# ktzsh/object-tracking

Measured on AMD Instinct MI355X. Metric: frames/sec detect+track @416x416, higher is better.
Workload: dtype f32; 1 GPU; BASELINE.json configs[2]: MultiObjDetTracker (YOLOv2 C=12 + ConvLSTM2D(512) + 1x1 + decode/NMS + track ids), 48 clips x 30 frames per GPU per step, 416x416 uint8; the synthetic head is calibrated to 32 CANDIDATE boxes per frame, of which about 20 survive NMS (config.boxes_per_frame: measured).  The step computes the model's TRACKING output, the one MultiObjDetTracker.predict reads (MultiObjDetTrac; parallelism=clip-shard x1

## Files before the change

### object_tracking_amd/csrc/conv3_h2.hip

```cpp
#include "dt_internal.h"
#include <type_traits>

typedef _Float16 c3_h8 __attribute__((ext_vector_type(8)));
typedef _Float16 c3_h4 __attribute__((ext_vector_type(4)));
typedef float c3_f16 __attribute__((ext_vector_type(16)));
typedef float c3_f4 __attribute__((ext_vector_type(4)));
typedef unsigned c3_u4 __attribute__((ext_vector_type(4)));
typedef unsigned c3_u2 __attribute__((ext_vector_type(2)));
typedef __attribute__((address_space(3))) void c3_lptr_t;
typedef const __attribute__((address_space(1))) void c3_gptr_t;

constexpr int C3_PW = 18;
#define C3_THREADS 256
#define C3_NS 3

template <int N>
__device__ __forceinline__ void c3_wait_vm() { __builtin_amdgcn_s_waitcnt(0x0f70 | (N & 15) | ((N >> 4) << 14)); }

__device__ __forceinline__ void c3_mfma(c3_f16 &c, const c3_u4 &w, const c3_u4 &a)
{
    c = __builtin_amdgcn_mfma_f32_32x32x16_f16(__builtin_bit_cast(c3_h8, a), __builtin_bit_cast(c3_h8, w), c, 0, 0, 0);
}

template <int WN, bool POOL, bool FUSE = false>
// ... 337 lines not shown
                            const float mx = fmaxf(fmaxf(acc[j][i][r], acc[j][i][r + 1]), fmaxf(acc[j][i][r + 8], acc[j][i][r + 9]));
                            const int x2 = (cur.tx0 >> 1) + 4 * (q >> 1) + 2 * gl + (q & 1);
                            if (nok && y2 < H2 && x2 < W2) {
                                if (p.amax_out) out_am = fmaxf(out_am, fabsf(mx));
                                __builtin_nontemporal_store(mx, p.out2 + (((long long)cur.b * H2 + y2) * W2 + x2) * p.out2_ld + cur.n0 + nl);
                            }
                        }
                    }
                }
            }
        }
        if (!has_next) break;
        __builtin_amdgcn_s_waitcnt(0xc07f);
        __builtin_amdgcn_s_barrier();
        patch_store();
        if (last_chunk && nxt.n0 != cur.n0)
            for (int i = tid; i < BN; i += C3_THREADS) btab[i] = (nxt.n0 + i < p.N) ? p.bias[nxt.n0 + i] : 0.0f;
        item = nitem;
        cur = nxt;
    }
    if (p.amax_out) dt_amax_publish(p.amax_out, out_am);
}

bool conv3_h2_usable(const Conv3H2Args &a)
{
    return a.Cin % 32 == 0 && a.Cin >= 32 && a.N >= 64 && a.N % 64 == 0 && a.Np % 64 == 0 && a.in_ld % 4 == 0 && (reinterpret_cast<uintptr_t>(a.in) & 15) == 0 &&
           a.w && a.pscale && a.amax && a.bias && a.zeros && (a.out != nullptr) != (a.out2 != nullptr) && (!a.out2 || !((a.H | a.W) & 1)) &&
           (!a.w1 || (a.N == 128 && a.out && a.pscale1 && a.bias1 && a.N1 > 0 && a.N1 <= 64 && a.Np1 >= 64 && a.Np1 % 32 == 0));
}
double conv3_h2_flops(const Conv3H2Args &a)
{
    const bool wide = a.N % 128 == 0;
    const int th = wide ? 8 : 16;
    const double tiles = (double)a.B * ((a.H + th - 1) / th) * ((a.W + 15) / 16);
    return 6.0 * tiles * th * 16 * (9.0 * a.Cin * a.N + (a.w1 ? (double)a.N * 64 : 0.0));
}

template <int WN, bool POOL, bool FUSE = false>
static int c3_launch(hipStream_t st, const Conv3H2Args &a, int cus)
{
    constexpr int TH = 16 / WN, BN = 64 * WN;
    const size_t lds = (size_t)4 * (TH + 2) * C3_PW * 32 + (size_t)C3_NS * 4 * BN * 32 + BN * 4 + (FUSE ? 68 * 4 : 0);
    static PerDeviceOnce attr;
    if (attr.ensure(nullptr, [&](int) {
            return hipFuncSetAttribute(reinterpret_cast<const void *>(conv3_h2_kernel<WN, POOL, FUSE>), hipFuncAttributeMaxDynamicSharedMemorySize, (int)lds) != hipSuccess;
        }))
        return 1;
    Conv3H2Args p = a;
    p.tiles_y = (a.H + TH - 1) / TH;
    p.tiles_x = (a.W + 15) / 16;
    const long long items = (long long)a.B * p.tiles_x * p.tiles_y * ((a.N + BN - 1) / BN);
    long long grid = 2ll * cus;
    if (grid > items) grid = items;
    hipLaunchKernelGGL((conv3_h2_kernel<WN, POOL, FUSE>), dim3((unsigned)grid), dim3(C3_THREADS), lds, st, p);
    return hipGetLastError() == hipSuccess ? 0 : 1;
}

int launch_conv3_h2(hipStream_t st, const Conv3H2Args &a)
{
    if (!conv3_h2_usable(a) || a.B <= 0 || a.H <= 0 || a.W <= 0) return 2;
    static int cu_of[64];
    static PerDeviceOnce once;
    int dev = 0;
    if (once.ensure(&dev, [&](int d) {
            int n = 0;
            if (hipDeviceGetAttribute(&n, hipDeviceAttributeMultiprocessorCount, d) != hipSuccess || n <= 0) return 1;
            cu_of[d] = n;
            return 0;
        }))
        return 1;
    const int cus = cu_of[dev];
    const bool wide = a.N % 128 == 0, pool = a.out2 != nullptr;
    if (a.w1) return c3_launch<2, false, true>(st, a, cus);
    if (wide) return pool ? c3_launch<2, true>(st, a, cus) : c3_launch<2, false>(st, a, cus);
    return pool ? c3_launch<1, true>(st, a, cus) : c3_launch<1, false>(st, a, cus);
}
```

### object_tracking_amd/csrc/dt_internal.h

```cpp
#pragma once
#include <hip/hip_runtime.h>

#include <atomic>
#include <cstdint>
#include <cstdio>
#include <map>
#include <mutex>
#include <functional>
#include <string>
#include <type_traits>
#include <vector>

#include "../../include/mi355_dt.h"

struct PerDeviceOnce {
    std::atomic<unsigned long long> mask{0};
    std::mutex mu;
    template <class F> int ensure(int *dev_out, F &&setup)
    {
        int dev = -1;
        if (hipGetDevice(&dev) != hipSuccess || dev < 0 || dev > 63) return 1;
        if (dev_out) *dev_out = dev;
        if ((mask.load(std::memory_order_acquire) >> dev) & 1ull) return 0;
        std::lock_guard<std::mutex> lk(mu);
// ... 101 lines not shown
struct Conv3H2Args {
    const float *in;
    long long in_bs;
    int in_ld;
    int B, H, W, Cin, N, Np;
    const unsigned short *w;
    const float *pscale;
    const unsigned *amax;
    const float *bias;
    float slope;
    float *out;
    long long out_bs;
    int out_ld;
    float *out2;
    int out2_ld;
    const float *zeros;
    unsigned *amax_out;
    int tiles_x, tiles_y;
    const unsigned short *w1;
    const float *pscale1;
    const float *bias1;
    int N1, Np1;
    float slope1;
};
int launch_conv3_h2(hipStream_t st, const Conv3H2Args &a);
bool conv3_h2_usable(const Conv3H2Args &a);
double conv3_h2_flops(const Conv3H2Args &a);
struct GemmS3Args {
    const unsigned short *a;
    const float *a_f32;
    int a_ld;
    const unsigned short *b;
    float *c;
    long long c_ps;
    int P, Mt, Mp, N, Np, K, ldc;
    const unsigned short *ones, *bias_s3;
    int act;
    float slope;
    int half;
    int nt;
    const float *pscale;
    const unsigned *amax;
    const float *bias;
    unsigned *amax_out;
};
#define DT_AMAX_SUB 16
// ... 342 lines not shown
    T *get() const { return p; }
    explicit operator bool() const { return p != nullptr; }
};
static_assert(!std::is_copy_constructible<DevMem<float>>::value && !std::is_copy_assignable<DevMem<float>>::value, "a device allocation has one owner");

struct WinoWeights {
    int ts = 0;
    int cin = 0, npad = 0;
    DevMem<float> u;
    DevMem<unsigned short> s3;
    DevMem<unsigned short> h2;
    DevMem<float> h2_pscale;
};

struct ConvLayer {
    int idx = 0, ks = 0, cin = 0, cout = 0, npad = 0;
    DevMem<float> wt;
    DevMem<unsigned short> wt_s3;
    DevMem<unsigned short> bias_s3;
    DevMem<unsigned short> wt_h2;
    DevMem<float> pscale_h2;
    DevMem<unsigned short> w3_h2;
    DevMem<float> pscale_w3;
    WinoWeights wino;
    WinoWeights wino_alt;
    DevMem<float> fused4s;
    DevMem<float> bias;
    DevMem<float> scale;
    bool scale_has_zero = false;
};

struct Policy {
    int wino = 1;
    int wino_tile = 0;
    int wino_mint = 0;
    double wino_ws_gb = 96.0;
    int mosaic = -1;
    int fused4 = 1;
    int trk_merge = 1;
    int pin = 0;
    int c3h2 = 1;
    int conv_cfg = -1;
    int s3_conv1 = 1;
    int s3 = 1;
    int s3_minrows = 2048;
    int s3_minrows_h2 = 64;
    int s3_h2 = 1;
    int c3fuse = 1;
    int h2_minframes = 12;
    int s3_half = 0;
    int s3_rec_minrows = 512;
    int s3_rec_minrows_h2 = 16;
    int s3_1x1_mink = 256;
    int s3_1x1_minrows = 16384;
    int s3_1x1 = 1;
    int amax_measure = 0;
};

struct StreamTable {
    int n_slots = 0, cap = 0;
    int tcap = 0;
    int row = 0;
    DevMem<float> h, c;
    DevMem<float> boxes;
// ... 1 lines not shown
    DevMem<int> ages;
    DevMem<float> vel;
    DevMem<int> vstamp;
    DevMem<int> hits;
    DevMem<int> hstamp;
    DevMem<int> meta;
    DevMem<int> list;
    std::vector<char> warm;
};

struct TinyStreamTable {
    int n_slots = 0;
    int U = 0;
    DevMem<float> h;
    DevMem<float> c;
    DevMem<int> meta;
    DevMem<int> list;
};

struct dt_ctx {
    std::string err;
    Policy pol;
    int pin_override = -1;
    hipStream_t stream = nullptr;
    int image_h = 0, image_w = 0, cb = 0;
    float dec_anchors_host[64];
    int dec_anchors_n = 0;
    bool det_loaded = false;
    ConvLayer layers[24];
    DevMem<float> s3_ones;
    DevMem<unsigned> amax;
    struct AmaxTag { const float *lo, *hi; int cols, slot; };
    bool h2_small = false;
    std::vector<AmaxTag> amax_tag;
    DevMem<float> conv1_w, conv1_b, lut255;
    DevMem<unsigned> conv1_w3, conv1_w3u8;
    std::vector<float> conv1_hwio32, conv1_scale, conv1_shift;
    bool trk_loaded = false;
    int trk_units = 0, trk_cx = 0 ;
    DevMem<float> trk_wx, trk_bx;
    DevMem<float> trk_wh;
    WinoWeights trk_wx_wino, trk_wh_wino;
    WinoWeights trk_wxm_wino;
    DevMem<float> trk_bx16;
    std::vector<float> conv23_hwio, conv23_bias;
    std::vector<float> trk_hkernel, trk_hbias;
// ... 41 lines not shown
```

### object_tracking_amd/csrc/network.hip

```cpp
#include <algorithm>
#include <cmath>
#include <cstdarg>
#include <cstdlib>
#include <cstring>
#include <thread>

#include "dt_internal.h"

static const float BN_EPS = 1e-3f;
static const float LEAKY = 0.1f;
static char g_static_err[512] = "";

static const int TRUNK[20][5] = {
    {1, 3, 3, 32, 1},      {2, 3, 32, 64, 1},     {3, 3, 64, 128, 0},    {4, 1, 128, 64, 0},
    {5, 3, 64, 128, 1},    {6, 3, 128, 256, 0},   {7, 1, 256, 128, 0},   {8, 3, 128, 256, 1},
    {9, 3, 256, 512, 0},   {10, 1, 512, 256, 0},  {11, 3, 256, 512, 0},  {12, 1, 512, 256, 0},
    {13, 3, 256, 512, 1},  {14, 3, 512, 1024, 0}, {15, 1, 1024, 512, 0}, {16, 3, 512, 1024, 0},
    {17, 1, 1024, 512, 0}, {18, 3, 512, 1024, 0}, {19, 3, 1024, 1024, 0}, {20, 3, 1024, 1024, 0}};

static inline int round_up(int v, int m) { return (v + m - 1) / m * m; }

int dt_fail(dt_ctx *ctx, int code, const char *fmt, ...)
{
    char buf[512];
// ... 204 lines not shown
    if (slot > AMAX_IN && slot < AMAX_TRK) snprintf(tag, sizeof(tag), "conv_%d", slot - AMAX_IN);
    else snprintf(tag, sizeof(tag), "%s", slot == AMAX_TRK ? "trk" : "test");
    ProfScope ps(ctx, "absmax", 0.0, 4.0 * (double)rows * cols, tag);
    if (launch_absmax(ctx->stream, x, rows, cols, ld, 1, 0, s)) { dt_fail(ctx, DT_ERR_DEVICE, "absmax launch failed"); return nullptr; }
    for (const auto &t : ctx->amax_tag)
        if (t.slot == slot) { amax_forget(ctx, t.lo, t.hi - t.lo); break; }
    amax_note(ctx, x, rows * ld, cols, slot);
    return s;
}
static bool h2_wanted(const dt_ctx *ctx) { return ctx->pol.s3 != 0 && ctx->pol.s3_h2 != 0 && !ctx->pol.pin && !ctx->h2_small; }

template <class T> static int upload(dt_ctx *ctx, DevMem<T> &dst, const std::vector<T> &h)
{
    DevMem<T> d;
    HIP_TRY(ctx, d.alloc(h.size()));
    HIP_TRY(ctx, hipMemcpy(d.get(), h.data(), h.size() * sizeof(T), hipMemcpyHostToDevice));
    dst = std::move(d);
    return DT_OK;
}

static const struct { const char *name; int Policy::*field; } k_knobs[] = {
    {"DT_WINO", &Policy::wino}, {"DT_WINO_TILE", &Policy::wino_tile}, {"DT_WINO_MINT", &Policy::wino_mint},
    {"DT_WINO_MOSAIC", &Policy::mosaic}, {"DT_WINO_FUSED4", &Policy::fused4}, {"DT_TRK_MERGE", &Policy::trk_merge},
    {"DT_PIN", &Policy::pin}, {"DT_C3H2", &Policy::c3h2}, {"DT_C3FUSE", &Policy::c3fuse}, {"DT_CONV_CFG", &Policy::conv_cfg},
    {"DT_S3", &Policy::s3}, {"DT_S3_CONV1", &Policy::s3_conv1}, {"DT_S3_MINROWS", &Policy::s3_minrows}, {"DT_S3_H2", &Policy::s3_h2},
    {"DT_H2_MINFRAMES", &Policy::h2_minframes}, {"DT_S3_HALF", &Policy::s3_half}, {"DT_S3_REC_MINROWS", &Policy::s3_rec_minrows},
    {"DT_S3_1X1", &Policy::s3_1x1}, {"DT_S3_1X1_MINK", &Policy::s3_1x1_mink}, {"DT_S3_1X1_MINROWS", &Policy::s3_1x1_minrows},
    {"DT_AMAX_MEASURE", &Policy::amax_measure},
};

static void policy_from_env(Policy &p)
{
    const Policy d;
    for (const auto &k : k_knobs) {
        const char *e = getenv(k.name);
        p.*k.field = e ? atoi(e) : d.*k.field;
    }
    { const char *e = getenv("DT_WINO_WS_GB"); p.wino_ws_gb = e ? atof(e) : d.wino_ws_gb; }
    p.s3_minrows_h2 = getenv("DT_S3_MINROWS") ? p.s3_minrows : d.s3_minrows_h2;
    p.s3_rec_minrows_h2 = getenv("DT_S3_REC_MINROWS") ? p.s3_rec_minrows : d.s3_rec_minrows_h2;
}

static bool policy_equal(const Policy &a, const Policy &b)
{
    for (const auto &k : k_knobs)
        if (a.*k.field != b.*k.field) return false;
    return a.wino_ws_gb == b.wino_ws_gb && a.s3_minrows_h2 == b.s3_minrows_h2 && a.s3_rec_minrows_h2 == b.s3_rec_minrows_h2;
}

static void policy_refresh(dt_ctx *ctx)
{
    Policy p;
    policy_from_env(p);
    if (ctx->pin_override >= 0) p.pin = ctx->pin_override;
    if (p.pin) {
        p.wino = 2; p.mosaic = 1; p.fused4 = 2; p.s3_half = -1;
        if (p.s3) p.s3 = 2;
        p.trk_merge = 0;
    }
    if (!policy_equal(p, ctx->pol)) graphs_clear(ctx);
    ctx->pol = p;
}

extern "C" int dt_abi_version(void) { return 108; }

extern "C" int dt_amax_read(dt_ctx *ctx, int slot, float *h_out)
{
    if (!ctx || !h_out) return dt_fail(ctx, DT_ERR_ARG, "null argument");
    if (slot < 0 || slot >= DT_AMAX_SLOTS) return dt_fail(ctx, DT_ERR_ARG, "max-|x| slot %d out of range [0, %d)", slot, DT_AMAX_SLOTS);
    if (!ctx->amax) return dt_fail(ctx, DT_ERR_STATE, "max-|x| slots not allocated");
    if (ctx->capturing) return dt_fail(ctx, DT_ERR_STATE, "dt_amax_read during graph capture");
    HIP_TRY(ctx, hipStreamSynchronize(ctx->stream));
    unsigned w[DT_AMAX_WORDS];
    HIP_TRY(ctx, hipMemcpy(w, amax_slot(ctx, slot), sizeof(w), hipMemcpyDeviceToHost));
    unsigned v = 0;
    for (int q = 0; q < DT_AMAX_SUB; ++q) v = w[q * DT_AMAX_LINE] > v ? w[q * DT_AMAX_LINE] : v;
    memcpy(h_out, &v, sizeof(v));
// ... 252 lines not shown
            wino_s3_split_host(bias_src[n], t);
            for (int t3 = 0; t3 < 3; ++t3) bs[((size_t)t3 * L.npad + n) * 16] = t[t3];
        }
        if ((rc = upload(ctx, L.bias_s3, bs))) return rc;
        if (!ctx->s3_ones) {
            std::vector<float> ones((size_t)256 * 16, 0.0f);
            for (int r = 0; r < 256; ++r) ones[(size_t)r * 16] = 1.0f;
            if ((rc = upload(ctx, ctx->s3_ones, ones))) return rc;
        }
    }
    if (L.wt_s3 && ctx->pol.s3_h2 != 0) {
        HIP_TRY(ctx, L.wt_h2.alloc(packed.size() * 2));
        HIP_TRY(ctx, L.pscale_h2.alloc(1));
        if (launch_wino_h2_pack(ctx->stream, L.wt.get(), 1, L.npad, cin, 0, amax_slot(ctx, AMAX_PACK), L.wt_h2.get(), L.pscale_h2.get()))
            return dt_fail(ctx, DT_ERR_DEVICE, "fp16-form weight pack launch failed");
        HIP_TRY(ctx, hipStreamSynchronize(ctx->stream));
    }
    if (ks == 3 && (cin == 32 || cin == 64) && cout % 64 == 0 && cout <= 128 && ctx->pol.s3 != 0 && ctx->pol.s3_h2 != 0 && ctx->pol.c3h2 != 0) {
        HIP_TRY(ctx, L.w3_h2.alloc(packed.size() * 2));
        HIP_TRY(ctx, L.pscale_w3.alloc(1));
        if (launch_wino_h2_pack(ctx->stream, L.wt.get(), 1, L.npad, 9 * cin, 0, amax_slot(ctx, AMAX_PACK), L.w3_h2.get(), L.pscale_w3.get()))
            return dt_fail(ctx, DT_ERR_DEVICE, "fp16-form weight pack launch failed");
        HIP_TRY(ctx, hipStreamSynchronize(ctx->stream));
    }
    if (scale) {
        std::vector<float> sc(scale, scale + cout);
        for (float v : sc) L.scale_has_zero |= (v == 0.0f);
        if ((rc = upload(ctx, L.scale, sc))) return rc;
    }
    const bool f4_shape = ((cin == 64 || cin == 128) && cout % 128 == 0 && cout <= 256) || (cin == 32 && cout == 64);
    if (ks == 3 && f4_shape && ctx->pol.wino != 0 && ctx->pol.fused4 != 0) {
        std::vector<float> u36((size_t)36 * L.npad * cin), uf((size_t)36 * cin * cout);
        wino_pack_weights(4, hwio, cin, cout, nullptr, cin, nullptr, L.npad, scale, u36.data());
        wino4s_fused_pack(u36.data(), L.npad, cin, cout, uf.data());
        if ((rc = upload(ctx, L.fused4s, uf))) return rc;
    }
    if (wino_wanted(ctx, ks, cin, cout)) {
        const int ts = wino_tile(ctx, false);
        rc = upload_wino(ctx, L.wino, ts, hwio, cin, cout, nullptr, cin, nullptr, L.npad, scale, ts == 6);
        if (rc) return rc;
        if (ts == 6 && ctx->pol.wino_tile == 0 && cin >= 256) {
            rc = upload_wino(ctx, L.wino_alt, 4, hwio, cin, cout, nullptr, cin, nullptr, L.npad, scale, false);
            if (rc) return rc;
        }
    }
    if ((rc = upload(ctx, L.bias, bias))) return rc;
// ... 333 lines not shown
{
    if (cout <= 64) return CFG_128x64;
    if (ks == 3 && cout % 256 == 0) {
        const long long t256 = (long long)((M + 255) / 256) * (cout / 256);
        const long long t128 = (long long)((M + 127) / 128) * (cout / 128);
        const double e256 = (double)t256 / (double)(((t256 + 255) / 256) * 256);
        const double e128 = (double)t128 / (double)(((t128 + 511) / 512) * 512);
        if (e256 * 1.05 > e128) return CFG_256x256;
    }
    if (ks == 1 && cout >= 128 && (long long)((M + 255) / 256) * ((cout + 127) / 128) >= 4096) return CFG_256x128;
    return CFG_128x128;
}

static bool s3_1x1_eligible(const dt_ctx *ctx, const ConvLayer &L, long long M)
{
    return L.ks == 1 && L.wt_s3 && ctx->pol.s3 != 0 && ctx->pol.s3_1x1 != 0 && L.cin % 32 == 0 && L.cout >= 64 && M < (1ll << 31) - 256 &&
           (ctx->pol.s3 == 2 || (L.cin >= S3_MINK && L.cin >= ctx->pol.s3_1x1_mink && M >= ctx->pol.s3_minrows && M >= ctx->pol.s3_1x1_minrows));
}

enum { CF_S3_1X1, CF_DIRECT_H2, CF_FUSED4, CF_WINO, CF_SPLITK, CF_IGEMM };
struct ConvChoice {
    int form;
    bool h2;
    int cfg, ksplit;
    const WinoWeights *wts; WinoChoice wino;
    bool publishes;
};
static ConvChoice choose_conv(const dt_ctx *ctx, const ConvLayer &L, const float *in, int in_ld, int B, int H, int W, const float *out, int order, int epi, bool has_out2)
{
    ConvChoice c{};
    const bool plain = epi == EPI_PLAIN && order == ORD_LINEAR, pool_even = epi == EPI_POOL && !((H | W) & 1);
    const long long blocks = (long long)B * ((H + 15) / 16) * ((W + 15) / 16) * ((L.cout + 127) / 128);
    if (L.bias_s3 && ctx->s3_ones && plain && !has_out2 && in_ld % 4 == 0 && (reinterpret_cast<uintptr_t>(in) & 15) == 0 &&
        (reinterpret_cast<uintptr_t>(out) & 3) == 0 && s3_1x1_eligible(ctx, L, (long long)B * H * W)) {
        c.form = CF_S3_1X1;
        c.h2 = L.wt_h2 && L.pscale_h2 && L.npad <= 2048 && h2_wanted(ctx);
    }
    else if (L.w3_h2 && L.pscale_w3 && ctx->pol.c3h2 != 0 && h2_wanted(ctx) && in_ld % 4 == 0 && (reinterpret_cast<uintptr_t>(in) & 15) == 0 && (plain || pool_even) &&
             (ctx->pol.c3h2 == 2 || blocks >= C3H2_MIN_BLOCKS))
        c.form = CF_DIRECT_H2;
    else if (L.fused4s && ctx->pol.fused4 != 0 && in_ld % 4 == 0 && (plain || pool_even) &&
             (ctx->pol.fused4 == 2 || (((ctx->pol.fused4 == 1 && L.cin <= 64) || ctx->pol.fused4 == 3) && blocks >= 1024)))
        c.form = CF_FUSED4;
    else if (wino_runs(ctx, L.wino, B, H, W, L.cout) && (plain || epi == EPI_POOL || epi == EPI_POOL_BOTH)) {
        const bool pooled = epi == EPI_POOL || has_out2;
        c.form = CF_WINO; c.wts = &L.wino;
        c.wino = choose_wino(ctx, L.wino, L.cout, B, H, W, pooled, false);
        if (L.wino_alt.u && !ctx->pol.pin) {
            const WinoChoice alt = choose_wino(ctx, L.wino_alt, L.cout, B, H, W, pooled, false);
            const long long t6 = 64ll * ((c.wino.q.Mt + 127) / 128) * ((L.cout + 127) / 128);
            if (c.wino.nt != 2 && t6 <= 4096 && small_gemm_cost(alt.q.Mt, L.cout, 36, nullptr) < small_gemm_cost(c.wino.q.Mt, L.cout, 64, nullptr)) {
                c.wts = &L.wino_alt; c.wino = alt;
            }
        }
    } else {
        const int M = B * H * W;
        c.form = CF_IGEMM; c.ksplit = 1;
        c.cfg = pick_cfg(M, L.cout, L.ks);
        if (plain && c.cfg != CFG_128x64) {
            const int tiles = ((M + 127) / 128) * ((L.cout + 127) / 128), nk = L.ks * L.ks * L.cin / 32;
            if (tiles < 2 * 512 && !ctx->pol.pin) {
                int smax = nk / 6;
                if (smax > 32) smax = 32;
// ... 17 lines not shown
    const ConvLayer &L; const float *in; int in_ld, B, H, W; float *out; int out_ld, order, epi; float slope; float *out2; int out2_ld;
    const char *tag; unsigned *amax_out; int M; double flops, bytes;
};

static int conv_s3_1x1(dt_ctx *ctx, const ConvCall &c, bool h2)
{
    const ConvLayer &L = c.L;
    const long long M = (long long)c.B * c.H * c.W;
    GemmS3Args g{};
    g.a_f32 = c.in; g.a_ld = c.in_ld; g.b = L.wt_s3.get(); g.c = c.out; g.c_ps = 0; g.P = 1; g.Mt = (int)M; g.Mp = (int)((M + 255) / 256 * 256); g.N = L.cout; g.Np = L.npad;
    g.half = ctx->pol.s3_half; g.K = L.cin; g.ldc = c.out_ld; g.ones = reinterpret_cast<const unsigned short *>(ctx->s3_ones.get()); g.bias_s3 = L.bias_s3.get(); g.act = 1; g.slope = c.slope;
    if (h2) {
        g.nt = 2; g.b = L.wt_h2.get(); g.pscale = L.pscale_h2.get(); g.bias = L.bias.get(); g.ones = nullptr; g.bias_s3 = nullptr;
        g.amax = ensure_amax(ctx, c.in, M, L.cin, c.in_ld, amax_in_slot(L));
        if (!g.amax) return DT_ERR_DEVICE;
    }
    g.amax_out = c.amax_out;
    prof_count(ctx, h2 ? "s3_form:f16x2" : "s3_form:bf16x3");
    ProfScope ps(ctx, "conv_gemm_s3", wino_gemm_s3_flops(g), 4.0 * M * L.cin + (h2 ? 4.0 : 6.0) * (double)L.cin * L.cout + 4.0 * (double)M * L.cout, c.tag);
    prof_direct_form(ctx, 2.0 * M * (double)L.cin * L.cout, 4.0 * ((double)M * L.cin + (double)L.cin * L.cout + (double)M * L.cout), DF_S3);
    const int rc = launch_wino_gemm_s3(ctx->stream, g, 0);
    return rc ? dt_fail(ctx, launch_code(rc), "%s: split-bf16 1x1 GEMM launch failed (rc=%d)", c.tag, rc) : DT_OK;
}
static int conv_direct_h2(dt_ctx *ctx, const ConvCall &c, const ConvLayer *L4 = nullptr)
{
    const ConvLayer &L = c.L;
    Conv3H2Args a{};
    a.in = c.in; a.in_bs = (long long)c.H * c.W * c.in_ld; a.in_ld = c.in_ld; a.B = c.B; a.H = c.H; a.W = c.W; a.Cin = L.cin; a.N = L.cout; a.Np = L.npad;
    a.w = L.w3_h2.get(); a.pscale = L.pscale_w3.get(); a.bias = L.bias.get(); a.slope = c.slope;
    if (L4) { a.w1 = L4->wt_h2.get(); a.pscale1 = L4->pscale_h2.get(); a.bias1 = L4->bias.get(); a.N1 = L4->cout; a.Np1 = L4->npad; a.slope1 = c.slope; }
    if (c.epi == EPI_POOL) { a.out2 = c.out; a.out2_ld = c.out_ld; }
    else { a.out = c.out; a.out_ld = c.out_ld; a.out_bs = (long long)c.H * c.W * c.out_ld; }
    a.zeros = ws_get(ctx, "zeros256", 256, true);
    if (!a.zeros) return DT_ERR_DEVICE;
    a.amax = ensure_amax(ctx, c.in, (long long)c.B * c.H * c.W, L.cin, c.in_ld, amax_in_slot(L));
    if (!a.amax) return DT_ERR_DEVICE;
    a.amax_out = c.amax_out;
    if (L4) prof_count(ctx, "conv_direct_h2:fused_1x1");
    const double M = c.M;
    ProfScope ps(ctx, "conv_direct_h2", conv3_h2_flops(a),
                 L4 ? 4.0 * (M * L.cin * 1.41 + M * L4->cout)
                    : 4.0 * ((double)c.B * c.H * c.W * L.cin * (L.cout % 128 ? 1.27 : 1.41) * ((L.cout + 127) / 128) + M * L.cout / (c.epi == EPI_POOL ? 4.0 : 1.0)), c.tag);
    if (L4)
        prof_direct_form(ctx, 2.0 * M * (9.0 * L.cin * L.cout + (double)L4->cin * L4->cout),
                         4.0 * (M * L.cin + 9.0 * L.cin * L.cout + 2.0 * M * L.cout + (double)L4->cin * L4->cout + M * L4->cout), DF_C3H2);
    else prof_direct_form(ctx, c.flops, c.bytes, DF_C3H2);
    const int rc = launch_conv3_h2(ctx->stream, a);
    return rc ? dt_fail(ctx, launch_code(rc), L4 ? "%s: fused direct 3x3 + 1x1 launch failed" : "%s: direct fp16-form 3x3 launch failed", c.tag) : DT_OK;
}
static int conv_fused4(dt_ctx *ctx, const ConvCall &c)
{
    const ConvLayer &L = c.L;
    Wino4FusedArgs f{};
    f.in = c.in; f.in_bs = (long long)c.H * c.W * c.in_ld; f.in_ld = c.in_ld; f.B = c.B; f.H = c.H; f.W = c.W; f.Cin = L.cin; f.N = L.cout;
    f.u = L.fused4s.get(); f.bias = L.bias.get(); f.slope = c.slope;
    if (c.epi == EPI_POOL) { f.out2 = c.out; f.out2_ld = c.out_ld; }
    else { f.out = c.out; f.out_ld = c.out_ld; f.out_bs = (long long)c.H * c.W * c.out_ld; }
    const double tiles = (double)c.B * ((c.H + 3) / 4) * ((c.W + 3) / 4);
    ProfScope ps(ctx, "conv_fused", 2.0 * 36.0 * tiles * L.cin * L.cout,
                 4.0 * ((double)c.B * c.H * c.W * L.cin * 1.27 * ((L.cout + 127) / 128) + (double)c.M * L.cout / (c.epi == EPI_POOL ? 4.0 : 1.0)), c.tag);
    prof_direct_form(ctx, c.flops, c.bytes, DF_FUSED);
// ... 37 lines not shown
            return dt_fail(ctx, DT_ERR_DEVICE, "conv_%d split-K reduce launch failed", L.idx);
        return DT_OK;
    }
    ProfScope ps(ctx, "conv_igemm", c.flops, c.bytes, c.tag);
    a.amax_out = c.amax_out;
    const int rc = launch_igemm(ctx, a, L.ks, c.order, c.epi, cfg);
    return rc ? dt_fail(ctx, launch_code(rc), "conv_%d launch failed (rc=%d)", L.idx, rc) : DT_OK;
}

static int run_conv(dt_ctx *ctx, const ConvLayer &L, const float *in, int in_ld, int B, int H, int W, float *out, int out_ld, int order, int epi, float slope,
                    float *out2 = nullptr, int out2_ld = 0)
{
    const Leaves lv = conv_leaves(epi, out, out_ld, out2, out2_ld, (long long)B * H * W, L.cout);
    amax_forget(ctx, lv);
    const ConvChoice ch = choose_conv(ctx, L, in, in_ld, B, H, W, out, order, epi, out2 != nullptr);
    const int M = B * H * W, K = L.ks * L.ks * L.cin;
    char tag[32];
    snprintf(tag, sizeof(tag), L.idx == 102 ? "tconv_2" : "conv_%d", L.idx);
    const ConvCall c{L, in, in_ld, B, H, W, out, out_ld, order, epi, slope, out2, out2_ld, tag, ch.publishes ? amax_slot(ctx, amax_out_slot(L)) : nullptr, M,
                     2.0 * M * (double)K * L.cout, 4.0 * ((double)M * L.cin + (double)K * L.cout + (double)M * L.cout / (epi == EPI_POOL ? 4.0 : 1.0))};
    int rc = DT_ERR_STATE;
    switch (ch.form) {
    case CF_S3_1X1: rc = conv_s3_1x1(ctx, c, ch.h2); break;
    case CF_DIRECT_H2: rc = conv_direct_h2(ctx, c); break;
    case CF_FUSED4: rc = conv_fused4(ctx, c); break;
    case CF_WINO: rc = conv_wino(ctx, c, *ch.wts, ch.wino); break;
    case CF_SPLITK: case CF_IGEMM: rc = conv_igemm(ctx, c, ch.cfg, ch.ksplit); break;
    }
    if (rc == DT_OK && c.amax_out) amax_note(ctx, lv, amax_out_slot(L));
    return rc;
}

enum { EX_CONV = 0, EX_NORM = 1, EX_ACT = 2, EX_POOL = 3, EX_S2D = 4, EX_CAT = 5 };
struct Extract {
    int idx, kind;
    float *out;
    bool done = false;
};

static int extract_layer(dt_ctx *ctx, const ConvLayer &L, const float *in, int in_ld, int B, int h, int w, Extract &ex)
{
    if (ex.kind == EX_CONV && L.scale && L.scale_has_zero)
        return dt_fail(ctx, DT_ERR_ARG, "conv_%d: a BatchNorm gamma of 0 was folded into the kernel; the raw Conv2D output cannot be recovered", L.idx);
    int rc = run_conv(ctx, L, in, in_ld, B, h, w, ex.out, L.cout, ORD_LINEAR, EPI_PLAIN, ex.kind == EX_ACT ? LEAKY : 1.0f);
    if (rc) return rc;
    if (ex.kind == EX_CONV && L.scale && launch_unfold_bn(ctx->stream, ex.out, (long long)B * h * w, L.cout, L.scale.get(), L.bias.get()))
        return dt_fail(ctx, DT_ERR_DEVICE, "BatchNorm un-fold launch failed");
    ex.done = true;
    return DT_OK;
}

static bool conv34_fusable(const dt_ctx *ctx, const ConvLayer &L3, const ConvLayer &L4, const float *in, int in_ld, int B, int H, int W, const float *out)
{
    return ctx->pol.c3fuse != 0 && L3.ks == 3 && L3.cout == 128 && L4.ks == 1 && L4.cin == 128 && L4.cout <= 64 && L4.wt_h2 && L4.pscale_h2 &&
           choose_conv(ctx, L3, in, in_ld, B, H, W, out, ORD_LINEAR, EPI_PLAIN, false).form == CF_DIRECT_H2;
}
static int run_conv34_fused(dt_ctx *ctx, const ConvLayer &L3, const ConvLayer &L4, const float *in, int in_ld, int B, int H, int W, float *out, int out_ld, float slope)
{
    const Leaves lv = conv_leaves(EPI_PLAIN, out, out_ld, nullptr, 0, (long long)B * H * W, L4.cout);
    amax_forget(ctx, lv);
    char tag[32];
    snprintf(tag, sizeof(tag), "conv_%d", L3.idx);
    const ConvCall c{L3, in, in_ld, B, H, W, out, out_ld, ORD_LINEAR, EPI_PLAIN, slope, nullptr, 0, tag, amax_out_slot(L4) ? amax_slot(ctx, amax_out_slot(L4)) : nullptr, B * H * W, 0.0, 0.0};
    const int rc = conv_direct_h2(ctx, c, &L4);
    if (rc == DT_OK && c.amax_out) amax_note(ctx, lv, amax_out_slot(L4));
    return rc;
}

static int run_trunk(dt_ctx *ctx, int B, float *bufA, float *bufB, float *skip, float *cat, Extract *ex)
{
    const int H = ctx->image_h, W = ctx->image_w;
    float *cur = bufA, *nxt = bufB;
    int h = H / 2, w = W / 2;
    int rc;
    bool cat20 = false;
    for (int li = 1; li < 20; ++li) {
        const int idx = TRUNK[li][0], pool = TRUNK[li][4];
        const ConvLayer &L = ctx->layers[idx];
        if (ex && ex->idx == idx && ex->kind <= EX_ACT) return extract_layer(ctx, L, cur, L.cin, B, h, w, *ex);
        if (idx == 3 && TRUNK[li + 1][0] == 4) {
            const bool ex4 = ex && ex->idx == 4;
            float *out34 = ex4 ? ex->out : nxt;
            if (!(ex4 && ex->kind < EX_ACT) && conv34_fusable(ctx, L, ctx->layers[4], cur, L.cin, B, h, w, out34)) {
                rc = run_conv34_fused(ctx, L, ctx->layers[4], cur, L.cin, B, h, w, out34, ctx->layers[4].cout, LEAKY);
                if (ex4) { ex->done = rc == DT_OK; return rc; }
                if (rc) return rc;
                float *t = cur; cur = nxt; nxt = t;
// ... 1407 lines not shown
    if (rows_form) { g.a = nullptr; g.a_f32 = d_v; g.a_ld = K; g.act = 1; g.slope = 1.0f; }
    g.c_ps = (long long)Mt * N; g.P = P; g.Mt = Mt; g.Mp = (int)Mp; g.N = N; g.Np = (int)Np; g.K = K; g.ldc = N; g.half = half;
    ProfScope pscope(ctx, "conv_gemm_s3", wino_gemm_s3_flops(g), (double)P * (2.0 * nt * Mt * K + 2.0 * nt * (double)K * N + 4.0 * (double)Mt * N), "test_gemm");
    if (pscope.on) prof_count(ctx, wino_gemm_s3_half_chosen(g, 0) ? "s3_tile:128x2" : "s3_tile:256");
    const int rc = launch_wino_gemm_s3(ctx->stream, g, 0);
    if (rc) return dt_fail(ctx, launch_code(rc), "dt_gemm_split: launch failed (rc=%d)", rc);
    return DT_OK;
}
extern "C" int dt_gemm_split_bf16(dt_ctx *ctx, const float *d_v, const float *d_u, int P, int Mt, int K, int N, int half, float *d_m)
{
    return dt_gemm_split(ctx, d_v, d_u, P, Mt, K, N, half, 3, d_m);
}

extern "C" int dt_policy_reload(dt_ctx *ctx)
{
    if (!ctx) return DT_ERR_ARG;
    policy_refresh(ctx);
    return DT_OK;
}

extern "C" int dt_policy_set(dt_ctx *ctx, const char *name, int value)
{
    if (!ctx || !name) return DT_ERR_ARG;
    if (strcmp(name, "pin") != 0) return dt_fail(ctx, DT_ERR_ARG, "dt_policy_set: unknown knob '%s'", name);
    if (value < -1 || value > 1) return dt_fail(ctx, DT_ERR_ARG, "dt_policy_set: pin must be -1, 0 or 1 (got %d)", value);
    ctx->pin_override = value;
    policy_refresh(ctx);
    return DT_OK;
}

static void prof_drain(dt_ctx *ctx)
{
    (void)hipStreamSynchronize(ctx->stream);
    for (auto &e : ctx->pending) {
        float ms = 0.0f;
        if (hipEventElapsedTime(&ms, e.a, e.b) == hipSuccess) {
            ctx->prof_tab[e.name].ms += ms;
            if (!e.tag.empty()) ctx->prof_tab[e.tag].ms += ms;
        }
        (void)hipEventDestroy(e.a);
        (void)hipEventDestroy(e.b);
    }
    ctx->pending.clear();
}

extern "C" int dt_profile_enable(dt_ctx *ctx, int on)
// ... 43 lines not shown
```

Baseline: 17360 frames/s.

## Add Winograd F(2,3)-along-y variant of direct fp16 3x3 conv kernel

Adds a new conv3x3 kernel that applies a 1-D Winograd F(2,3) transform along the y axis, cutting the MFMA multiply count per output from 9 to 6 taps per input channel. Transformed weights (12 per channel instead of 9) are precomputed at load time for 128-output-channel layers. The input patch is transformed on the fly before being split into hi/lo fp16 pairs, and the output inverse transform is fused into the epilogue, including the pool path. It is enabled by default for eligible layers through a new policy knob. The trade-off is more LDS and register pressure, extra transform arithmetic, and some change in numerical error.

```diff
diff --git a/object_tracking_amd/csrc/conv3_h2.hip b/object_tracking_amd/csrc/conv3_h2.hip
--- a/object_tracking_amd/csrc/conv3_h2.hip
+++ b/object_tracking_amd/csrc/conv3_h2.hip
@@ -383,8 +383,242 @@
     if (p.amax_out) dt_amax_publish(p.amax_out, out_am);
 }
 
+constexpr int WY_PLANE = 16 * C3_PW * 32;
+constexpr int WY_PATCH = 4 * WY_PLANE;
+constexpr int WY_BPL = 128 * 32, WY_BSTAGE = 4 * WY_BPL;
+constexpr int WY_NS = 2;
+constexpr int WY_NJ = 10;
+constexpr int WY_LDS = WY_PATCH + WY_NS * WY_BSTAGE + 128 * 4;
+
+template <bool POOL>
+__global__ __launch_bounds__(C3_THREADS) __attribute__((amdgpu_waves_per_eu(2, 2))) void conv3_h2_wy_kernel(Conv3H2Args p)
+{
+    constexpr int TH = 8, TW = 16, BN = 128, PW = C3_PW, PLANE = WY_PLANE, BPL = WY_BPL, BSTAGE = WY_BSTAGE, PB = 4, NJ = WY_NJ;
+    extern __shared__ __attribute__((aligned(16))) unsigned char c3_lds[];
+    unsigned char *patch = c3_lds, *bring = c3_lds + WY_PATCH;
+    float *btab = reinterpret_cast<float *>(c3_lds + WY_PATCH + WY_NS * BSTAGE);
+    const int tid = threadIdx.x, lane = tid & 63, wave = tid >> 6;
+    const int wm = wave & 1, wn = wave >> 1;
+    const int rl = lane & 31, gl = lane >> 5;
+
+    const unsigned am = dt_amax_read(p.amax);
+    const float fwd = dt_h2_base(am) * 0.5f;
+    const float inv = p.pscale[0] * dt_h2_base_inv(am) * 2.0f;
+    const int nchunk = p.Cin >> 5;
+    const int ntn = (p.N + BN - 1) / BN;
+    const int tiles = p.tiles_x * p.tiles_y;
+    const long long items = (long long)p.B * tiles * ntn;
+    const long long wterm = (long long)(12 * p.Cin / 16) * p.Np * 16;
+    float out_am = 0.0f;
+
+    long long item = blockIdx.x;
+    if (item >= items) return;
+
+    struct Unit { int b, ty0, tx0, n0, chunk; };
+    auto unit_of = [&](long long it, int chunk) {
+        Unit u;
+        u.n0 = (int)(it % ntn) * BN;
+        const long long r = it / ntn;
+        const int t = (int)(r % tiles);
+        u.b = (int)(r / tiles);
+        u.ty0 = (t / p.tiles_x) * TH;
+        u.tx0 = (t % p.tiles_x) * TW;
+        u.chunk = chunk;
+        return u;
+    };
+    const int ppx = tid >> 3, pc4 = tid & 7;
+    const bool pact = tid < 18 * 8;
+    c3_f4 pf[NJ];
+    auto patch_request = [&](const Unit &u) {
+        const int x = u.tx0 + ppx - 1;
+        const bool xok = pact && x >= 0 && x < p.W;
+        const float *col = p.in + (long long)u.b * p.in_bs + (long long)x * p.in_ld + u.chunk * 32 + pc4 * 4;
+#pragma unroll
+        for (int j = 0; j < NJ; ++j) {
+            const int y = u.ty0 + j - 1;
+            const bool ok = xok && y >= 0 && y < p.H;
+            const float *src = ok ? col + (long long)y * p.W * p.in_ld : p.zeros;
+            pf[j] = *reinterpret_cast<const c3_f4 *>(src);
+        }
+    };
+    auto patch_store = [&]() {
+        if (pact) {
+            const int half = pc4 >> 2;
+            int lbase = ppx * 32 + ((pc4 >> 1) & 1) * 16 + (pc4 & 1) * 8 + (half * 2) * PLANE;
+            asm volatile("" : "+v"(lbase));
+#pragma unroll
+            for (int q = 0; q < 4; ++q) {
+                const c3_f4 d0 = pf[2 * q], d1 = pf[2 * q + 1], d2 = pf[2 * q + 2], d3 = pf[2 * q + 3];
+                const c3_f4 t[4] = {d0 - d2, d1 + d2, d2 - d1, d1 - d3};
+#pragma unroll
+                for (int pos = 0; pos < 4; ++pos) {
+                    const int a0 = lbase + (pos * 4 + q) * PW * 32;
+                    const c3_f4 x = t[pos] * fwd;
+                    const c3_h4 hi = __builtin_convertvector(x, c3_h4);
+                    const c3_f4 r = x - __builtin_convertvector(hi, c3_f4);
+                    const c3_h4 lo = __builtin_convertvector(r, c3_h4);
+                    unsigned char *dst = patch + (a0 ^ ((a0 >> 4) & 16));
+                    *reinterpret_cast<c3_u2 *>(dst) = __builtin_bit_cast(c3_u2, hi);
+                    *reinterpret_cast<c3_u2 *>(dst + PLANE) = __builtin_bit_cast(c3_u2, lo);
+                }
+            }
+        }
+    };
+    const int lrow = lane >> 1;
+    const int dgran = (lane & 1) ^ ((lrow >> 3) & 1);
+    const unsigned short *wsrc = p.w + (wave & 1) * wterm + ((long long)(wave >> 1) * p.Np + lrow) * 16 + dgran * 8;
+    const int wdst = wave * BPL;
+    const long long wstage = (long long)2 * p.Np * 16;
+    auto stage_off = [&](int n0, int chunk, int s) { return (long long)(chunk * 12 + s) * wstage + (long long)n0 * 16; };
+    auto piece_issue = [&](int buf, long long off, int q) {
+        __builtin_amdgcn_global_load_lds((c3_gptr_t *)(wsrc + off + q * 512), (c3_lptr_t *)(bring + buf * BSTAGE + wdst + q * 1024), 16, 0, 0);
+    };
+    int offB[2];
+#pragma unroll
+    for (int j = 0; j < 2; ++j) {
+        const int row = wn * 64 + 32 * j + rl;
+        offB[j] = (2 * row + (gl ^ ((row >> 3) & 1))) * 16;
+    }
+    int pixA = (2 * wm + (rl >> 4)) * PW + (rl & 15);
+    auto offA_of = [&](int s) {
+        const int pix = pixA + (s / 3) * 4 * PW + s % 3;
+        return pix * 32 + ((gl ^ ((pix >> 3) & 1)) * 16);
+    };
+
+    Unit cur = unit_of(item, 0);
+    patch_request(cur);
+#pragma unroll
+    for (int q = 0; q < PB; ++q) piece_issue(0, stage_off(cur.n0, 0, 0), q);
+    for (int i = tid; i < BN; i += C3_THREADS) btab[i] = (cur.n0 + i < p.N) ? p.bias[cur.n0 + i] : 0.0f;
+    patch_store();
+
+    c3_f16 acc[4][2];
+    c3_u4 fa[2][2], fb[2][2][2];
+    for (;;) {
+        asm volatile("" : "+v"(pixA));
+        if (cur.chunk == 0) {
+#pragma unroll
+            for (int pos = 0; pos < 4; ++pos)
+#pragma unroll
+                for (int j = 0; j < 2; ++j)
+#pragma unroll
+                    for (int e = 0; e < 16; ++e) acc[pos][j][e] = 0.0f;
+        }
+        const bool last_chunk = cur.chunk == nchunk - 1;
+        const long long nitem = last_chunk ? item + gridDim.x : item;
+        const bool has_next = nitem < items;
+        Unit nxt = cur;
+        if (has_next) nxt = unit_of(nitem, last_chunk ? 0 : cur.chunk + 1);
+
+        auto stage = [&](auto sc) {
+            constexpr int s = decltype(sc)::value;
+            constexpr int pos = s / 3;
+            if (s == 1 && has_next) c3_wait_vm<NJ>();
+            else c3_wait_vm<0>();
+            __builtin_amdgcn_s_waitcnt(0xc07f);
+            __builtin_amdgcn_s_barrier();
+            const bool refill = s < 11 || has_next;
+            const long long roff = s < 11 ? stage_off(cur.n0, cur.chunk, s + 1) : stage_off(nxt.n0, nxt.chunk, 0);
+            const unsigned char *sb = bring + (s & 1) * BSTAGE;
+#pragma unroll
+            for (int j = 0; j < 2; ++j)
+#pragma unroll
+                for (int t = 1; t >= 0; --t) fb[0][j][t] = *reinterpret_cast<const c3_u4 *>(sb + t * BPL + offB[j]);
+            if (s == 0) {
+#pragma unroll
+                for (int t = 0; t < 2; ++t) fa[0][t] = *reinterpret_cast<const c3_u4 *>(patch + t * PLANE + offA_of(0));
+            }
+            const int oa = offA_of(s), on = offA_of(s < 11 ? s + 1 : 0);
+            __builtin_amdgcn_sched_barrier(0);
+#pragma unroll
+            for (int hf = 0; hf < 2; ++hf) {
+#pragma unroll
+                for (int m = 0; m < 6; ++m) {
+                    const int pr = m >> 1, j = m & 1;
+                    c3_mfma(acc[pos][j], fb[hf][j][pr == 0 ? 1 : 0], fa[hf][pr == 1 ? 1 : 0]);
+                    if (hf == 0) {
+                        if (m == 0 || m == 3) fa[1][m == 3] = *reinterpret_cast<const c3_u4 *>(patch + (2 + (m == 3)) * PLANE + oa);
+                        else { const int jb = (m == 2 || m == 5), tb = m < 3; fb[1][jb][tb] = *reinterpret_cast<const c3_u4 *>(sb + (2 + tb) * BPL + offB[jb]); }
+                        if (m < PB && refill) piece_issue((s + 1) & 1, roff, m);
+                    } else if (s < 11 && m < 2) {
+                        fa[0][m] = *reinterpret_cast<const c3_u4 *>(patch + m * PLANE + on);
+                    }
+                    __builtin_amdgcn_sched_barrier(0);
+                }
+                if (s == 0 && hf == 0 && has_next) { patch_request(nxt); __builtin_amdgcn_sched_barrier(0); }
+            }
+        };
+        stage(std::integral_constant<int, 0>{}); stage(std::integral_constant<int, 1>{}); stage(std::integral_constant<int, 2>{});
+        stage(std::integral_constant<int, 3>{}); stage(std::integral_constant<int, 4>{}); stage(std::integral_constant<int, 5>{});
+        stage(std::integral_constant<int, 6>{}); stage(std::integral_constant<int, 7>{}); stage(std::integral_constant<int, 8>{});
+        stage(std::integral_constant<int, 9>{}); stage(std::integral_constant<int, 10>{}); stage(std::integral_constant<int, 11>{});
+
+        if (last_chunk) {
+#pragma unroll
+            for (int j = 0; j < 2; ++j)
+#pragma unroll
+                for (int e = 0; e < 16; ++e) {
+                    const float m0 = acc[0][j][e], m1 = acc[1][j][e], m2 = acc[2][j][e], m3 = acc[3][j][e];
+                    acc[0][j][e] = (m0 + m1) + m2;
+                    acc[1][j][e] = (m1 - m2) - m3;
+                }
+            int et = tid;
+            asm volatile("" : "+v"(et));
+            const int erl = et & 31, egl = (et >> 5) & 1;
+#pragma unroll
+            for (int j = 0; j < 2; ++j) {
+                const int nl = wn * 64 + 32 * j + erl;
+                const float bl = btab[nl];
+                const bool nok = cur.n0 + nl < p.N;
+#pragma unroll
+                for (int rr = 0; rr < 2; ++rr)
+#pragma unroll
+                    for (int e = 0; e < 16; ++e) {
+                        const float z = __builtin_fmaf(acc[rr][j][e], inv, bl);
+                        acc[rr][j][e] = fmaxf(z, z * p.slope);
+                    }
+                if (!POOL) {
+#pragma unroll
+                    for (int rr = 0; rr < 2; ++rr)
+#pragma unroll
+                        for (int e = 0; e < 16; ++e) {
+                            const int m = 8 * (e >> 2) + 4 * egl + (e & 3);
+                            const int y = cur.ty0 + 4 * wm + 2 * (m >> 4) + rr, x = cur.tx0 + (m & 15);
+                            if (nok && y < p.H && x < p.W) {
+                                if (p.amax_out) out_am = fmaxf(out_am, fabsf(acc[rr][j][e]));
+                                __builtin_nontemporal_store(acc[rr][j][e], p.out + (long long)cur.b * p.out_bs + ((long long)y * p.W + x) * p.out_ld + cur.n0 + nl);
+                            }
+                        }
+                } else {
+                    const int H2 = p.H >> 1, W2 = p.W >> 1;
+#pragma unroll
+                    for (int e = 0; e < 16; e += 2) {
+                        const int m = 8 * (e >> 2) + 4 * egl + (e & 3);
+                        const float mx = fmaxf(fmaxf(acc[0][j][e], acc[0][j][e + 1]), fmaxf(acc[1][j][e], acc[1][j][e + 1]));
+                        const int y2 = (cur.ty0 >> 1) + 2 * wm + (m >> 4), x2 = (cur.tx0 >> 1) + ((m & 15) >> 1);
+                        if (nok && y2 < H2 && x2 < W2) {
+                            if (p.amax_out) out_am = fmaxf(out_am, fabsf(mx));
+                            __builtin_nontemporal_store(mx, p.out2 + (((long long)cur.b * H2 + y2) * W2 + x2) * p.out2_ld + cur.n0 + nl);
+                        }
+                    }
+                }
+            }
+        }
+        if (!has_next) break;
+        __builtin_amdgcn_s_waitcnt(0xc07f);
+        __builtin_amdgcn_s_barrier();
+        patch_store();
+        if (last_chunk && nxt.n0 != cur.n0)
+            for (int i = tid; i < BN; i += C3_THREADS) btab[i] = (nxt.n0 + i < p.N) ? p.bias[nxt.n0 + i] : 0.0f;
+        item = nitem;
+        cur = nxt;
+    }
+    if (p.amax_out) dt_amax_publish(p.amax_out, out_am);
+}
+
 bool conv3_h2_usable(const Conv3H2Args &a)
 {
+    if (a.wy && (a.N % 128 != 0 || a.w1)) return false;
     return a.Cin % 32 == 0 && a.Cin >= 32 && a.N >= 64 && a.N % 64 == 0 && a.Np % 64 == 0 && a.in_ld % 4 == 0 && (reinterpret_cast<uintptr_t>(a.in) & 15) == 0 &&
            a.w && a.pscale && a.amax && a.bias && a.zeros && (a.out != nullptr) != (a.out2 != nullptr) && (!a.out2 || !((a.H | a.W) & 1)) &&
            (!a.w1 || (a.N == 128 && a.out && a.pscale1 && a.bias1 && a.N1 > 0 && a.N1 <= 64 && a.Np1 >= 64 && a.Np1 % 32 == 0));
@@ -394,7 +628,7 @@
     const bool wide = a.N % 128 == 0;
     const int th = wide ? 8 : 16;
     const double tiles = (double)a.B * ((a.H + th - 1) / th) * ((a.W + 15) / 16);
-    return 6.0 * tiles * th * 16 * (9.0 * a.Cin * a.N + (a.w1 ? (double)a.N * 64 : 0.0));
+    return 6.0 * tiles * th * 16 * ((a.wy ? 6.0 : 9.0) * a.Cin * a.N + (a.w1 ? (double)a.N * 64 : 0.0));
 }
 
 template <int WN, bool POOL, bool FUSE = false>
@@ -417,6 +651,24 @@
     return hipGetLastError() == hipSuccess ? 0 : 1;
 }
 
+template <bool POOL>
+static int c3_launch_wy(hipStream_t st, const Conv3H2Args &a, int cus)
+{
+    static PerDeviceOnce attr;
+    if (attr.ensure(nullptr, [&](int) {
+            return hipFuncSetAttribute(reinterpret_cast<const void *>(conv3_h2_wy_kernel<POOL>), hipFuncAttributeMaxDynamicSharedMemorySize, WY_LDS) != hipSuccess;
+        }))
+        return 1;
+    Conv3H2Args p = a;
+    p.tiles_y = (a.H + 7) / 8;
+    p.tiles_x = (a.W + 15) / 16;
+    const long long items = (long long)a.B * p.tiles_x * p.tiles_y * ((a.N + 127) / 128);
+    long long grid = 2ll * cus;
+    if (grid > items) grid = items;
+    hipLaunchKernelGGL((conv3_h2_wy_kernel<POOL>), dim3((unsigned)grid), dim3(C3_THREADS), WY_LDS, st, p);
+    return hipGetLastError() == hipSuccess ? 0 : 1;
+}
+
 int launch_conv3_h2(hipStream_t st, const Conv3H2Args &a)
 {
     if (!conv3_h2_usable(a) || a.B <= 0 || a.H <= 0 || a.W <= 0) return 2;
@@ -432,6 +684,7 @@
         return 1;
     const int cus = cu_of[dev];
     const bool wide = a.N % 128 == 0, pool = a.out2 != nullptr;
+    if (a.wy) return pool ? c3_launch_wy<true>(st, a, cus) : c3_launch_wy<false>(st, a, cus);
     if (a.w1) return c3_launch<2, false, true>(st, a, cus);
     if (wide) return pool ? c3_launch<2, true>(st, a, cus) : c3_launch<2, false>(st, a, cus);
     return pool ? c3_launch<1, true>(st, a, cus) : c3_launch<1, false>(st, a, cus);
diff --git a/object_tracking_amd/csrc/dt_internal.h b/object_tracking_amd/csrc/dt_internal.h
--- a/object_tracking_amd/csrc/dt_internal.h
+++ b/object_tracking_amd/csrc/dt_internal.h
@@ -147,6 +147,7 @@
     const float *bias1;
     int N1, Np1;
     float slope1;
+    int wy;
 };
 int launch_conv3_h2(hipStream_t st, const Conv3H2Args &a);
 bool conv3_h2_usable(const Conv3H2Args &a);
@@ -535,6 +536,8 @@
     DevMem<float> pscale_h2;
     DevMem<unsigned short> w3_h2;
     DevMem<float> pscale_w3;
+    DevMem<unsigned short> w3_wy;
+    DevMem<float> pscale_wy;
     WinoWeights wino;
     WinoWeights wino_alt;
     DevMem<float> fused4s;
@@ -553,6 +556,7 @@
     int trk_merge = 1;
     int pin = 0;
     int c3h2 = 1;
+    int c3h2_wy = 1;
     int conv_cfg = -1;
     int s3_conv1 = 1;
     int s3 = 1;
@@ -600,6 +604,7 @@
     std::string err;
     Policy pol;
     int pin_override = -1;
+    int c3h2_wy_override = -1;
     hipStream_t stream = nullptr;
     int image_h = 0, image_w = 0, cb = 0;
     float dec_anchors_host[64];
diff --git a/object_tracking_amd/csrc/network.hip b/object_tracking_amd/csrc/network.hip
--- a/object_tracking_amd/csrc/network.hip
+++ b/object_tracking_amd/csrc/network.hip
@@ -250,7 +250,7 @@
 static const struct { const char *name; int Policy::*field; } k_knobs[] = {
     {"DT_WINO", &Policy::wino}, {"DT_WINO_TILE", &Policy::wino_tile}, {"DT_WINO_MINT", &Policy::wino_mint},
     {"DT_WINO_MOSAIC", &Policy::mosaic}, {"DT_WINO_FUSED4", &Policy::fused4}, {"DT_TRK_MERGE", &Policy::trk_merge},
-    {"DT_PIN", &Policy::pin}, {"DT_C3H2", &Policy::c3h2}, {"DT_C3FUSE", &Policy::c3fuse}, {"DT_CONV_CFG", &Policy::conv_cfg},
+    {"DT_PIN", &Policy::pin}, {"DT_C3H2", &Policy::c3h2}, {"DT_C3H2_WY", &Policy::c3h2_wy}, {"DT_C3FUSE", &Policy::c3fuse}, {"DT_CONV_CFG", &Policy::conv_cfg},
     {"DT_S3", &Policy::s3}, {"DT_S3_CONV1", &Policy::s3_conv1}, {"DT_S3_MINROWS", &Policy::s3_minrows}, {"DT_S3_H2", &Policy::s3_h2},
     {"DT_H2_MINFRAMES", &Policy::h2_minframes}, {"DT_S3_HALF", &Policy::s3_half}, {"DT_S3_REC_MINROWS", &Policy::s3_rec_minrows},
     {"DT_S3_1X1", &Policy::s3_1x1}, {"DT_S3_1X1_MINK", &Policy::s3_1x1_mink}, {"DT_S3_1X1_MINROWS", &Policy::s3_1x1_minrows},
@@ -281,6 +281,7 @@
     Policy p;
     policy_from_env(p);
     if (ctx->pin_override >= 0) p.pin = ctx->pin_override;
+    if (ctx->c3h2_wy_override >= 0) p.c3h2_wy = ctx->c3h2_wy_override;
     if (p.pin) {
         p.wino = 2; p.mosaic = 1; p.fused4 = 2; p.s3_half = -1;
         if (p.s3) p.s3 = 2;
@@ -579,6 +580,25 @@
         if (launch_wino_h2_pack(ctx->stream, L.wt.get(), 1, L.npad, 9 * cin, 0, amax_slot(ctx, AMAX_PACK), L.w3_h2.get(), L.pscale_w3.get()))
             return dt_fail(ctx, DT_ERR_DEVICE, "fp16-form weight pack launch failed");
         HIP_TRY(ctx, hipStreamSynchronize(ctx->stream));
+        if (cout == 128 && ctx->pol.c3h2_wy != 0) {
+            const int K9 = 9 * cin, K12 = 12 * cin;
+            std::vector<float> wy((size_t)L.npad * K12);
+            for (int n = 0; n < L.npad; ++n)
+                for (int ci = 0; ci < cin; ++ci)
+                    for (int kx = 0; kx < 3; ++kx) {
+                        const float *row = packed.data() + (size_t)n * K9 + (size_t)(ci / 32) * 9 * 32 + ci % 32;
+                        const double g0 = row[(0 * 3 + kx) * 32], g1 = row[(1 * 3 + kx) * 32], g2 = row[(2 * 3 + kx) * 32];
+                        const double u[4] = {g0, (g0 + g1 + g2) / 2, (g0 - g1 + g2) / 2, g2};
+                        for (int pos = 0; pos < 4; ++pos) wy[(size_t)n * K12 + ((size_t)((ci / 32) * 4 + pos) * 3 + kx) * 32 + ci % 32] = (float)u[pos];
+                    }
+            DevMem<float> wy_dev;
+            if ((rc = upload(ctx, wy_dev, wy))) return rc;
+            HIP_TRY(ctx, L.w3_wy.alloc(wy.size() * 2));
+            HIP_TRY(ctx, L.pscale_wy.alloc(1));
+            if (launch_wino_h2_pack(ctx->stream, wy_dev.get(), 1, L.npad, K12, 0, amax_slot(ctx, AMAX_PACK), L.w3_wy.get(), L.pscale_wy.get()))
+                return dt_fail(ctx, DT_ERR_DEVICE, "fp16-form weight pack launch failed");
+            HIP_TRY(ctx, hipStreamSynchronize(ctx->stream));
+        }
     }
     if (scale) {
         std::vector<float> sc(scale, scale + cout);
@@ -958,6 +978,7 @@
 struct ConvChoice {
     int form;
     bool h2;
+    bool wy;
     int cfg, ksplit;
     const WinoWeights *wts; WinoChoice wino;
     bool publishes;
@@ -973,8 +994,10 @@
         c.h2 = L.wt_h2 && L.pscale_h2 && L.npad <= 2048 && h2_wanted(ctx);
     }
     else if (L.w3_h2 && L.pscale_w3 && ctx->pol.c3h2 != 0 && h2_wanted(ctx) && in_ld % 4 == 0 && (reinterpret_cast<uintptr_t>(in) & 15) == 0 && (plain || pool_even) &&
-             (ctx->pol.c3h2 == 2 || blocks >= C3H2_MIN_BLOCKS))
+             (ctx->pol.c3h2 == 2 || blocks >= C3H2_MIN_BLOCKS)) {
         c.form = CF_DIRECT_H2;
+        c.wy = L.cout == 128 && L.w3_wy && L.pscale_wy && (ctx->pol.c3h2_wy == 2 || (ctx->pol.c3h2_wy == 1 && blocks >= C3H2_MIN_BLOCKS));
+    }
     else if (L.fused4s && ctx->pol.fused4 != 0 && in_ld % 4 == 0 && (plain || pool_even) &&
              (ctx->pol.fused4 == 2 || (((ctx->pol.fused4 == 1 && L.cin <= 64) || ctx->pol.fused4 == 3) && blocks >= 1024)))
         c.form = CF_FUSED4;
@@ -1038,12 +1061,14 @@
     const int rc = launch_wino_gemm_s3(ctx->stream, g, 0);
     return rc ? dt_fail(ctx, launch_code(rc), "%s: split-bf16 1x1 GEMM launch failed (rc=%d)", c.tag, rc) : DT_OK;
 }
-static int conv_direct_h2(dt_ctx *ctx, const ConvCall &c, const ConvLayer *L4 = nullptr)
+static int conv_direct_h2(dt_ctx *ctx, const ConvCall &c, bool wy, const ConvLayer *L4 = nullptr)
 {
     const ConvLayer &L = c.L;
+    if (wy && (L4 || !L.w3_wy || !L.pscale_wy)) return dt_fail(ctx, DT_ERR_STATE, "%s: the F(2,3)-along-y form was chosen for a launch it cannot take", c.tag);
     Conv3H2Args a{};
     a.in = c.in; a.in_bs = (long long)c.H * c.W * c.in_ld; a.in_ld = c.in_ld; a.B = c.B; a.H = c.H; a.W = c.W; a.Cin = L.cin; a.N = L.cout; a.Np = L.npad;
     a.w = L.w3_h2.get(); a.pscale = L.pscale_w3.get(); a.bias = L.bias.get(); a.slope = c.slope;
+    if (wy) { a.w = L.w3_wy.get(); a.pscale = L.pscale_wy.get(); a.wy = 1; }
     if (L4) { a.w1 = L4->wt_h2.get(); a.pscale1 = L4->pscale_h2.get(); a.bias1 = L4->bias.get(); a.N1 = L4->cout; a.Np1 = L4->npad; a.slope1 = c.slope; }
     if (c.epi == EPI_POOL) { a.out2 = c.out; a.out2_ld = c.out_ld; }
     else { a.out = c.out; a.out_ld = c.out_ld; a.out_bs = (long long)c.H * c.W * c.out_ld; }
@@ -1053,6 +1078,7 @@
     if (!a.amax) return DT_ERR_DEVICE;
     a.amax_out = c.amax_out;
     if (L4) prof_count(ctx, "conv_direct_h2:fused_1x1");
+    prof_count(ctx, wy ? "c3h2_form:wy" : "c3h2_form:direct");
     const double M = c.M;
     ProfScope ps(ctx, "conv_direct_h2", conv3_h2_flops(a),
                  L4 ? 4.0 * (M * L.cin * 1.41 + M * L4->cout)
@@ -1136,7 +1162,7 @@
     int rc = DT_ERR_STATE;
     switch (ch.form) {
     case CF_S3_1X1: rc = conv_s3_1x1(ctx, c, ch.h2); break;
-    case CF_DIRECT_H2: rc = conv_direct_h2(ctx, c); break;
+    case CF_DIRECT_H2: rc = conv_direct_h2(ctx, c, ch.wy); break;
     case CF_FUSED4: rc = conv_fused4(ctx, c); break;
     case CF_WINO: rc = conv_wino(ctx, c, *ch.wts, ch.wino); break;
     case CF_SPLITK: case CF_IGEMM: rc = conv_igemm(ctx, c, ch.cfg, ch.ksplit); break;
@@ -1176,7 +1202,7 @@
     char tag[32];
     snprintf(tag, sizeof(tag), "conv_%d", L3.idx);
     const ConvCall c{L3, in, in_ld, B, H, W, out, out_ld, ORD_LINEAR, EPI_PLAIN, slope, nullptr, 0, tag, amax_out_slot(L4) ? amax_slot(ctx, amax_out_slot(L4)) : nullptr, B * H * W, 0.0, 0.0};
-    const int rc = conv_direct_h2(ctx, c, &L4);
+    const int rc = conv_direct_h2(ctx, c, false, &L4);
     if (rc == DT_OK && c.amax_out) amax_note(ctx, lv, amax_out_slot(L4));
     return rc;
 }
@@ -2630,6 +2656,12 @@
 extern "C" int dt_policy_set(dt_ctx *ctx, const char *name, int value)
 {
     if (!ctx || !name) return DT_ERR_ARG;
+    if (strcmp(name, "c3h2_wy") == 0) {
+        if (value < -1 || value > 2) return dt_fail(ctx, DT_ERR_ARG, "dt_policy_set: c3h2_wy must be -1, 0, 1 or 2 (got %d)", value);
+        ctx->c3h2_wy_override = value;
+        policy_refresh(ctx);
+        return DT_OK;
+    }
     if (strcmp(name, "pin") != 0) return dt_fail(ctx, DT_ERR_ARG, "dt_policy_set: unknown knob '%s'", name);
     if (value < -1 || value > 1) return dt_fail(ctx, DT_ERR_ARG, "dt_policy_set: pin must be -1, 0 or 1 (got %d)", value);
     ctx->pin_override = value;
```

Result: faster. 17550 frames/s, median of 6 (+1.1%).
